# halide/Halide

Measured on AMD Instinct MI355X. Metric: megapixels/sec local_laplacian 8-level fp32 4K, higher is better.
Workload: dtype f32; 1 GPU; apps/local_laplacian J=8 levels=8 alpha=1/7 beta=1, u16 RGB planar 3840x2160; distinct_frames_per_gpu=8, lut_cached=True, streams_per_gpu=4, frame_scheduling=4 frame-queue streams, boundary=C ABI local_laplacian(halide_buffer_t*,int32,float,float,halide_buffer_t*), rccl_ranks=1, parallelism=frames sharded over 1 GPU(s), no data-path collective

## Files before the change

halide_amd/csrc/local_laplacian.hip:

```cpp
#include "hlmi_device_math.h"
#include "hlmi_internal.h"

#include <atomic>
#include <mutex>
#include <optional>
#include <stdlib.h>
#include <string.h>
#include <type_traits>

using namespace hlmi;

namespace {

constexpr int J = 8;
constexpr int MAX_K = 32;
constexpr int STRIP = 126;
constexpr int KCH = 8;
constexpr int D0_THREADS = 256;

struct Level {
    int lox, loy;
    int w, h;
    int ws;
    size_t ps;
// ... 55 lines not shown
    if (i > 2 * half) return;
    float fx = (float)(i - half) * (1.0f / 256.0f);
    lut[i] = (alpha * fx) * dev::halide_exp(((-fx) * fx) * 0.5f);
}

__device__ __forceinline__ int xcd_block() {
    const int nb8 = gridDim.x >> 3, b = blockIdx.x;
    return (b < (nb8 << 3)) ? (b & 7) * nb8 + (b >> 3) : b;
}

__device__ __forceinline__ float down4(float a, float b, float c, float d) {
    return (dev::mad(3.0f, b + c, a) + d) * 0.125f;
}
__device__ __forceinline__ float down4_raw(float a, float b, float c, float d) { return dev::mad(3.0f, b + c, a) + d; }
__device__ __forceinline__ float down4_tail(float a, float b, float c, float d) {
    return (dev::mad(3.0f, b + c, a) + d) * 0.015625f;
}

__device__ __forceinline__ float gray_from(uint16_t r, uint16_t g, uint16_t b) {
    constexpr float s = (float)(1.0 / 65535.0);
    constexpr float C0 = (float)((double)s * (double)0.299f), C1 = (float)((double)s * (double)0.587f),
                    C2 = (float)((double)s * (double)0.114f);
    return dev::mad((float)b, C2, dev::mad2((float)r, C0, (float)g, C1));
}
__device__ __forceinline__ int idx_of(float gray, float Km1, int half) {
    return dev::clampi((int)((gray * Km1) * 256.0f), 0, half);
}
template<bool B1 = false>
__device__ __forceinline__ float g0_val(float gray, float level, float beta, float l) {
    return B1 ? ((gray - level) + level) + l : dev::mad(beta, gray - level, level) + l;
}

__device__ __forceinline__ float lane_prev(float v) {
    return __builtin_bit_cast(float, __builtin_amdgcn_update_dpp(0, __builtin_bit_cast(int, v), 0x138, 0xf, 0xf, true));
}
__device__ __forceinline__ float lane_next(float v) {
    return __builtin_bit_cast(float, __builtin_amdgcn_update_dpp(0, __builtin_bit_cast(int, v), 0x130, 0xf, 0xf, true));
}
__global__ void ll_dpp_probe(int *ok) {
    float v = (float)threadIdx.x;
    float p = lane_prev(v), n = lane_next(v);
    bool good = (threadIdx.x == 0 || p == v - 1.0f) && (threadIdx.x == 63 || n == v + 1.0f);
    unsigned long long m = __ballot(good);
    if (threadIdx.x == 0) *ok = (m == ~0ull) ? 1 : 0;
}

template<bool ODD>
__device__ __forceinline__ float2 hpair(const float (&dy)[4]) {
    if (!ODD) {
        float left = lane_prev(dy[3]);
        float right = lane_next(dy[0]);
        float o0 = down4_tail(left, dy[0], dy[1], dy[2]);
        float o1 = down4_tail(dy[1], dy[2], dy[3], right);
        float o2 = lane_next(o0);
        return make_float2(o1, o2);
    } else {
        float r0 = lane_next(dy[0]), r1 = lane_next(dy[1]);
        float o0 = down4_tail(dy[0], dy[1], dy[2], dy[3]);
        float o1 = down4_tail(dy[2], dy[3], r0, r1);
        return make_float2(o0, o1);
    }
}

struct QuadSel {
    int oq;
    int sel[4];
    bool plain;
};
__device__ __forceinline__ QuadSel quad_sel(int o, int w) {
    QuadSel q;
    q.oq = dev::clampi(o, 0, (w - 1) & ~3);
#pragma unroll
    for (int i = 0; i < 4; i++) q.sel[i] = dev::clampi(o + i, 0, w - 1) - q.oq;
    q.plain = (o >= 0) && (o + 3 <= w - 1);
    return q;
}
template<typename T>
__device__ __forceinline__ T pick4(T x, T y, T z, T w, int s) {
    T lo = (s & 1) ? y : x, hi = (s & 1) ? w : z;
    return (s & 2) ? hi : lo;
}

typedef unsigned short us4_t __attribute__((ext_vector_type(4)));
template<bool NT = false>
__device__ __forceinline__ ushort4 ld_frame4(const uint16_t *p) {
    if (NT) {
        us4_t v = __builtin_nontemporal_load(reinterpret_cast<const us4_t *>(p));
        return make_ushort4(v.x, v.y, v.z, v.w);
    }
    return *reinterpret_cast<const ushort4 *>(p);
}
template<bool NT = false>
__device__ __forceinline__ ushort2 ld_frame2(const void *sbase, uint32_t byte_off) {
    const uint32_t *q = reinterpret_cast<const uint32_t *>(reinterpret_cast<const char *>(sbase) + byte_off);
    const uint32_t w = NT ? __builtin_nontemporal_load(q) : *q;
    return make_ushort2((uint16_t)(w & 0xffffu), (uint16_t)(w >> 16));
}
template<bool NT = false>
__device__ __forceinline__ void st_frame2(void *p, uint16_t a, uint16_t b) {
    const uint32_t w = (uint32_t)a | ((uint32_t)b << 16);
    if (NT) __builtin_nontemporal_store(w, reinterpret_cast<uint32_t *>(p));
    else *reinterpret_cast<uint32_t *>(p) = w;
}

struct Raw {
    ushort4 c0, c1, c2;
};
struct Levels {
    float v[MAX_K];
};

template<bool VEC, bool NT = false>
__device__ __forceinline__ void load_raw(Raw &r, const uint16_t *__restrict__ rp, long co0, long co1, long co2,
                                         int oq, const int (&xo)[4]) {
    if (VEC) {
        r.c0 = ld_frame4<NT>(rp + co0 + oq);
        r.c1 = ld_frame4<NT>(rp + co1 + oq);
        r.c2 = ld_frame4<NT>(rp + co2 + oq);
    } else {
        r.c0 = make_ushort4(rp[co0 + xo[0]], rp[co0 + xo[1]], rp[co0 + xo[2]], rp[co0 + xo[3]]);
        r.c1 = make_ushort4(rp[co1 + xo[0]], rp[co1 + xo[1]], rp[co1 + xo[2]], rp[co1 + xo[3]]);
        r.c2 = make_ushort4(rp[co2 + xo[0]], rp[co2 + xo[1]], rp[co2 + xo[2]], rp[co2 + xo[3]]);
    }
}

template<bool ODD, bool VEC, bool LUT_LDS, bool B1>
__global__ __launch_bounds__(D0_THREADS, 2) void ll_down0(const uint16_t *__restrict__ in, long in_sy, long co0, long co1,
                                                   long co2, Geometry gm, Levels lev, float beta,
                                                   const float *__restrict__ lut_g, float *__restrict__ g1, int Xs,
                                                   int loy1, int w1, int h1, int ws1, size_t ps1, int nsx, int nsy,
                                                   int nunits) {
    extern __shared__ float slut[];
    if (LUT_LDS) {
        for (int i = threadIdx.x; i <= 2 * gm.half; i += D0_THREADS) slut[i] = lut_g[i];
        __syncthreads();
    }
    const float *lut = LUT_LDS ? slut : lut_g;
    const int wave = __builtin_amdgcn_readfirstlane(threadIdx.x >> 6);
    const int unit = xcd_block() * (D0_THREADS / 64) + wave;
    if (unit >= nunits) return;
    const int lane = threadIdx.x & 63;
    const int sy = unit % nsy, sx = unit / nsy;
    const int off = STRIP * sx + 2 * lane;
    const int P = Xs + off;
    const int q0 = ODD ? 2 * P - 1 : 2 * P - 2;
    const int iw = gm.ix1 - gm.ix0 + 1, ih = gm.iy1 - gm.iy0;
    const QuadSel qs = quad_sel(q0 - gm.ix0, iw);
    int xo[4];
#pragma unroll
    for (int i = 0; i < 4; i++) xo[i] = qs.oq + qs.sel[i];
    const bool edge_wave = VEC && __any(!qs.plain);
    const bool store_ok = (lane < 63) && (off < w1);
    const int t0 = (int)((long)sy * h1 / nsy), t1 = (int)((long)(sy + 1) * h1 / nsy) - 1;

    auto row_ptr = [&](int y_abs) -> const uint16_t * {
        return in + (long)(dev::clampi(y_abs - gm.iy0, 0, ih)) * in_sy;
    };

    for (int kb = 0; kb < gm.K; kb += KCH) {
        const int nk = min(KCH, gm.K - kb);
        const bool with_in = (kb == 0);
        const int lbase = gm.half - 256 * (kb + KCH - 1);
        float level[KCH];
#pragma unroll
        for (int kk = 0; kk < KCH; kk++) {
            const float lk = (float)(kb + kk) * gm.inv_Km1;
// ... 353 lines not shown
                level2(kk - 1);
            }
            __builtin_amdgcn_sched_barrier(0);
        }
        state_issue(KCH);
        res[KCH] = hpair<ODD0>(dy[KCH & 1]);
        level2(KCH);
        prep_row(rc, n0);
        prep_row(rd, n1);
        __builtin_amdgcn_sched_barrier(0);
        if (T >= Ts0 && T <= Ts1) {
            float *drow = p.g1 + (size_t)(T - p.loy1) * p.ws1 + off1;
            if (st1_ok) {
#pragma unroll
                for (int kk = 0; kk <= KCH; kk++) *reinterpret_cast<float2 *>(drow + (size_t)kk * p.ps1) = res[kk];
            }
        }
        if (EXCH && pub) {
#pragma unroll
            for (int kk = 0; kk <= KCH; kk++) pub[kk * 64] = res[kk];
        }
        __builtin_amdgcn_sched_barrier(0);
        if (T + 1 < T1) {
            load_row(rc, 2 * T + 5);
            load_row(rd, 2 * T + 6);
        }
        __builtin_amdgcn_sched_barrier(0);
    };
    Row p0, p1, p2, p3;
    prep_row(rc, p0);
    prep_row(rd, p1);
    load_row(rc, 2 * T0 + 3);
    load_row(rd, 2 * T0 + 4);
    LL_PROBE_T(pt2);
    for (int T = T0; T <= T1; T += 2) {
        const bool first = EXCH && T == T0;
        step(std::integral_constant<int, 0>{}, T, p0, p1, p2, p3, a, b, a2, b2, first && publish ? pub_mine : nullptr);
        step(std::integral_constant<int, 1>{}, T + 1, p2, p3, p0, p1, a2, b2, a, b,
             first && publish ? pub_mine + (KCH + 1) * 64 : nullptr);
        if (first) __syncthreads();
#if HLMI_LL_PROBE
        if (first) { LL_PROBE_T(pt3); pr_3 = pt3; }
#endif
    }
    LL_PROBE_T(pt4);
    LL_PROBE_ADD(0, pt1 - pt0); LL_PROBE_ADD(1, 1); LL_PROBE_ADD(2, pt2 - pt1); LL_PROBE_ADD(3, pr_3 - pt2);
    LL_PROBE_ADD(16, pr_a - pr_a0); LL_PROBE_ADD(17, pr_a0 - pt1);
    LL_PROBE_ADD(4, pt4 - pt2); LL_PROBE_ADD(5, (T1 - T0 + 1)); LL_PROBE_ADD(6, pt4 - pt0);
    if (EXCH && !self_halo) {
        float *d2 = p.g2 + (size_t)(B - p.loy2) * p.ws2 + off2;
#pragma unroll
        for (int k = 0; k <= KCH; k++) {
            const float2 sa = st2[(2 * k) * 64], sb = st2[(2 * k + 1) * 64];
            const float2 c = pub_next[k * 64], d = pub_next[(KCH + 1 + k) * 64];
            const float rx = dev::mad(3.0f, sb.x + c.x, sa.x) + d.x, ry = dev::mad(3.0f, sb.y + c.y, sa.y) + d.y;
            float o;
            if (ODD1) {
                const float nx = lane_next(rx), ny = lane_next(ry);
                o = down4_tail(rx, ry, nx, ny);
            } else {
                const float py = lane_prev(ry), nx = lane_next(rx);
                o = down4_tail(py, rx, ry, nx);
            }
            if (st2_ok) d2[(size_t)k * p.ps2] = o;
        }
    }
    };
    if (edge_wave) walk(std::true_type{});
    else walk(std::false_type{});
}

struct D01EArgs {
    D01Args d;
    float *outl0;
    int oy0, oh;
    unsigned nsx_magic;
};
typedef float f2 __attribute__((ext_vector_type(2)));
__device__ __forceinline__ f2 f2s(float v) { return f2{v, v}; }
__device__ __forceinline__ f2 fma2(f2 a, f2 b, f2 c) { return __builtin_elementwise_fma(a, b, c); }
__device__ __forceinline__ f2 mad_2(f2 a, f2 b, f2 c) { return dev::CANON_FMA ? fma2(a, b, c) : a * b + c; }
__device__ __forceinline__ f2 mad2_2(f2 a, f2 b, f2 c, f2 d) { return dev::CANON_FMA ? fma2(a, b, c * d) : a * b + c * d; }

template<bool ODD0, bool ODD1, bool B1, bool EXCH, bool NT>
__global__ __launch_bounds__(D0_THREADS, 2) void ll_down01e(D01EArgs pe, Geometry gm, Levels lev) {
    const D01Args &p = pe.d;
    LL_RESIDENCY(0);
    extern __shared__ float slut[];
    for (int i = threadIdx.x; i <= 2 * gm.half; i += D0_THREADS) slut[i] = p.lut_g[i];
    __syncthreads();
    const int wave = __builtin_amdgcn_readfirstlane(threadIdx.x >> 6);
    const int lane = threadIdx.x & 63;
    int sx, A, B;
    bool self_halo = true;
    bool publish = false;
    if (EXCH) {
        const int wg = xcd_block();
        const int gy = pe.nsx_magic ? (int)__umulhi((unsigned)wg, pe.nsx_magic) : wg;
        sx = wg - gy * p.nsx;
        const int GA = p.loy2 + gy * p.rows_base + min(gy, p.rows_rem);
        const int GB = GA + p.rows_base + (gy < p.rows_rem ? 1 : 0) - 1;
        const int n = (GB - GA + 1 + 1 + 3) >> 2;
        A = GA + wave * n, B = min(A + n - 1, GB);
        if (A > GB) {
            __syncthreads();
            return;
        }
        self_halo = !(wave < 3 && A + n <= GB);
        publish = wave > 0;
    } else {
        const int unit = xcd_block() * (D0_THREADS / 64) + wave;
        if (unit >= p.nunits) return;
        sx = p.nsy_magic ? (int)__umulhi((unsigned)unit, p.nsy_magic) : unit;
        const int sy = unit - sx * p.nsy;
        A = p.loy2 + sy * p.rows_base + min(sy, p.rows_rem);
        B = A + p.rows_base + (sy < p.rows_rem ? 1 : 0) - 1;
    }
    const int P = p.Pbase + 2 * p.S2 * sx + 2 * lane;
    const int q0 = ODD0 ? 2 * P - 1 : 2 * P - 2;
    const int iw = gm.ix1 - gm.ix0 + 1, ih = gm.iy1 - gm.iy0;
    const QuadSel qs = quad_sel(q0 - gm.ix0, iw);
    int xo[4];
#pragma unroll
    for (int i = 0; i < 4; i++) xo[i] = qs.oq + qs.sel[i];
    const bool edge_wave = __any(!qs.plain);
    const int T0 = 2 * A - 1, T1 = self_halo ? 2 * B + 2 : 2 * B;
    const int Ts0 = max(EXCH ? 2 * A - 1 : 2 * A, p.loy1), Ts1 = min(EXCH ? 2 * B : 2 * B + 1, p.loy1 + p.h1 - 1);
    const int off1 = P - p.so1;
    const bool st1_ok = lane < p.S2 && off1 >= 0 && off1 < p.w1;
    const int X2 = ODD1 ? (P + 1) >> 1 : P >> 1;
    const int off2 = X2 - p.so2;
    const bool st2_ok = (ODD1 ? lane < p.S2 : (lane >= 1 && lane <= p.S2)) && off2 >= 0 && off2 < p.w2;
    const bool em_ok = lane >= 1 && lane <= p.S2 && q0 >= gm.ix0 && q0 + 3 <= gm.ix1;
    float *const em_col = pe.outl0 + (q0 - gm.ix0);
    f2 *st2 = reinterpret_cast<f2 *>(slut + ((2 * gm.half + 2) & ~1)) + wave * D01_STATE + lane;
    f2 *pub_all = reinterpret_cast<f2 *>(slut + ((2 * gm.half + 2) & ~1)) + (D0_THREADS / 64) * D01_STATE + lane;
    f2 *pub_mine = pub_all + (wave - 1) * D01_STATE, *pub_next = pub_all + wave * D01_STATE;
    const int lbase = gm.half - 256 * (KCH - 1);
    float level[KCH];
#pragma unroll
    for (int kk = 0; kk < KCH; kk++) {
        level[kk] = lev.v[kk];
        asm volatile("" : "+v"(level[kk]));
    }
    auto walk = [&](auto edge_tag) {
    constexpr bool EDGE = decltype(edge_tag)::value;
    auto load_row = [&](Raw &r, int y_abs) {
        const uint16_t *rp = p.in + (long)(dev::clampi(y_abs - gm.iy0, 0, ih)) * p.in_sy;
        load_raw<true, NT>(r, rp, p.co0, p.co1, p.co2, qs.oq, xo);
    };
    auto u16s = [&](const ushort4 &c, uint16_t (&o)[4]) {
        const uint2 w = __builtin_bit_cast(uint2, c);
        o[0] = (uint16_t)(w.x & 0xffffu), o[1] = (uint16_t)(w.x >> 16);
        o[2] = (uint16_t)(w.y & 0xffffu), o[3] = (uint16_t)(w.y >> 16);
    };
    struct Row {
        f2 g[2];
        int l[4];
    };
    auto prep_row = [&](const Raw &r, Row &o) {
        uint16_t rr[4], gg[4], bb[4];
        u16s(r.c0, rr), u16s(r.c1, gg), u16s(r.c2, bb);
        constexpr float s = (float)(1.0 / 65535.0);
        constexpr float C0 = (float)((double)s * (double)0.299f), C1 = (float)((double)s * (double)0.587f),
                        C2 = (float)((double)s * (double)0.114f);
#pragma unroll
        for (int h = 0; h < 2; h++) {
            const f2 fr = {(float)rr[h], (float)rr[h + 2]}, fg = {(float)gg[h], (float)gg[h + 2]}, fb = {(float)bb[h], (float)bb[h + 2]};
            o.g[h] = mad_2(fb, f2s(C2), mad2_2(fr, f2s(C0), fg, f2s(C1)));
        }
        if (EDGE) {
            const float g0 = o.g[0].x, g1v = o.g[1].x, g2v = o.g[0].y, g3 = o.g[1].y;
            o.g[0].x = pick4(g0, g1v, g2v, g3, qs.sel[0]), o.g[1].x = pick4(g0, g1v, g2v, g3, qs.sel[1]);
            o.g[0].y = pick4(g0, g1v, g2v, g3, qs.sel[2]), o.g[1].y = pick4(g0, g1v, g2v, g3, qs.sel[3]);
        }
#pragma unroll
        for (int h = 0; h < 2; h++) {
            const f2 t = (o.g[h] * gm.Km1) * 256.0f;
            o.l[h] = (min((int)t.x, gm.half) + lbase) * 4;
            o.l[h + 2] = (min((int)t.y, gm.half) + lbase) * 4;
        }
#pragma unroll
        for (int i = 0; i < 4; i++) asm volatile("" : "+v"(o.l[i]));
    };
    auto lut_issue = [&](int kk, const Row &r0, const Row &r1, f2 (&dst)[4]) {
        auto rd = [&](int l) {
            return *reinterpret_cast<const float *>(reinterpret_cast<const char *>(slut) + l + 1024 * (KCH - 1 - kk));
        };
        dst[0].x = rd(r0.l[0]), dst[1].x = rd(r0.l[1]), dst[0].y = rd(r0.l[2]), dst[1].y = rd(r0.l[3]);
        dst[2].x = rd(r1.l[0]), dst[3].x = rd(r1.l[1]), dst[2].y = rd(r1.l[2]), dst[3].y = rd(r1.l[3]);
    };
    auto plane_vals = [&](int kk, const Row &r0, const Row &r1, const f2 (&lv)[4], f2 (&v0)[2], f2 (&v1)[2]) {
        if (B1 && kk == 0) {
            v0[0] = r0.g[0] + lv[0], v0[1] = r0.g[1] + lv[1], v1[0] = r1.g[0] + lv[2], v1[1] = r1.g[1] + lv[3];
        } else if (kk < KCH) {
            const f2 L = f2s(level[kk < KCH ? kk : 0]);
            f2 t[4] = {r0.g[0] - L, r0.g[1] - L, r1.g[0] - L, r1.g[1] - L};
            if (!B1 && !dev::CANON_FMA) {
#pragma unroll
                for (int i = 0; i < 4; i++) t[i] = p.beta * t[i];
            }
#pragma unroll
            for (int i = 0; i < 4; i++) t[i] = (!B1 && dev::CANON_FMA) ? fma2(f2s(p.beta), t[i], L) : t[i] + L;
            v0[0] = t[0] + lv[0], v0[1] = t[1] + lv[1], v1[0] = t[2] + lv[2], v1[1] = t[3] + lv[3];
        } else {
            v0[0] = r0.g[0], v0[1] = r0.g[1], v1[0] = r1.g[0], v1[1] = r1.g[1];
        }
    };
    auto vpass = [&](const f2 (&ia)[2], const f2 (&ib)[2], const f2 (&c)[2], const f2 (&d)[2], f2 (&o)[2]) {
        f2 t[2] = {ib[0] + c[0], ib[1] + c[1]};
        if (dev::CANON_FMA) {
            t[0] = fma2(f2s(3.0f), t[0], ia[0]), t[1] = fma2(f2s(3.0f), t[1], ia[1]);
        } else {
            t[0] = 3.0f * t[0], t[1] = 3.0f * t[1];
            t[0] = ia[0] + t[0], t[1] = ia[1] + t[1];
        }
        o[0] = t[0] + d[0], o[1] = t[1] + d[1];
    };
    auto hpair2 = [&](const f2 (&dy)[2]) {
        const float d4[4] = {dy[0].x, dy[1].x, dy[0].y, dy[1].y};
        const float2 r = hpair<ODD0>(d4);
        return f2{r.x, r.y};
    };
    struct EmPix {
        f2 lut, qa, qb, ta, tb;
        float lif;
    };
    auto em_gather = [&](const Row &n, int i, const f2 *rq, const f2 *rt, EmPix &g) {
        constexpr int COL[4] = {ODD0 ? -1 : -2, -1, ODD0 ? 0 : -1, 0};
        const uint32_t aq0 = (uint32_t)(size_t)rq, at0 = (uint32_t)(size_t)rt, alut = (uint32_t)(size_t)slut + 1024u * (KCH - 2);
        auto rd2 = [](uint32_t addr, auto swap_tag) {
            f2 v;
            if (decltype(swap_tag)::value) asm volatile("ds_read2st64_b32 %0, %1 offset0:4" : "=v"(v) : "v"(addr) : "memory");
            else asm volatile("ds_read2st64_b32 %0, %1 offset1:4" : "=v"(v) : "v"(addr) : "memory");
            return v;
        };
        constexpr std::false_type asc{};
        constexpr std::true_type desc{};
        const int pos = n.l[i] - lbase * 4;
        const int li = min(pos >> 10, KCH - 2);
        const uint32_t po = (uint32_t)(li << 10) + (uint32_t)(COL[i] * 4);
        g.lut = rd2(alut + (uint32_t)n.l[i] - (uint32_t)(li << 10), desc);
        if ((COL[i] & 1) == 0) {
            auto rd64 = [](uint32_t addr, auto plane1) {
                f2 v;
                if (decltype(plane1)::value) asm volatile("ds_read_b64 %0, %1 offset:1024" : "=v"(v) : "v"(addr) : "memory");
                else asm volatile("ds_read_b64 %0, %1" : "=v"(v) : "v"(addr) : "memory");
                return v;
            };
            g.qa = rd64(aq0 + po, asc), g.qb = rd64(aq0 + po, desc);
            g.ta = rd64(at0 + po, asc), g.tb = rd64(at0 + po, desc);
        } else {
            g.qa = rd2(aq0 + po, asc), g.qb = rd2(aq0 + po + 4u, asc);
            g.ta = rd2(at0 + po, asc), g.tb = rd2(at0 + po + 4u, asc);
        }
        g.lif = (float)li;
    };
    auto em_wait = [&](EmPix &g, auto after_tag) {
        constexpr int AFTER = decltype(after_tag)::value;
        static_assert(AFTER >= 0 && AFTER <= 3, "");
        if (AFTER == 0) asm volatile("s_waitcnt lgkmcnt(0)" : "+v"(g.lut), "+v"(g.qa), "+v"(g.qb), "+v"(g.ta), "+v"(g.tb));
        if (AFTER == 1) asm volatile("s_waitcnt lgkmcnt(5)" : "+v"(g.lut), "+v"(g.qa), "+v"(g.qb), "+v"(g.ta), "+v"(g.tb));
        if (AFTER == 2) asm volatile("s_waitcnt lgkmcnt(10)" : "+v"(g.lut), "+v"(g.qa), "+v"(g.qb), "+v"(g.ta), "+v"(g.tb));
        if (AFTER == 3) asm volatile("s_waitcnt lgkmcnt(15)" : "+v"(g.lut), "+v"(g.qa), "+v"(g.qb), "+v"(g.ta), "+v"(g.tb));
    };
    auto em_arith = [&](const Row &n, int i, const EmPix &g, auto yodd_tag) {
        constexpr bool YODD = decltype(yodd_tag)::value;
        const bool xodd = ODD0 ? (i & 1) == 0 : (i & 1) == 1;
        auto hl = [&](f2 fa, f2 fb) {
            if (xodd) return fma2(fb, f2s(0.25f), fa * 0.75f);
            return dev::CANON_FMA ? fma2(fb, f2s(0.75f), fa * 0.25f) : fma2(fa, f2s(0.25f), fb * 0.75f);
        };
        auto vl = [](f2 uq, f2 ut) {
            return (dev::CANON_FMA && !YODD) ? fma2(ut, f2s(0.75f), uq * 0.25f) : fma2(uq, f2s(0.25f), ut * 0.75f);
        };
        const float gr = n.g[i & 1][i >> 1];
        const float lf = gr * gm.Km1 - g.lif;
        const f2 lev = f2{g.lif, g.lif + 1.0f} * gm.inv_Km1;
        constexpr int COLP[4] = {ODD0 ? -1 : -2, -1, ODD0 ? 0 : -1, 0};
        f2 u;
        if ((COLP[i] & 1) == 0) {
            auto hls = [&](float fa, float fb) {
                if (xodd) return __builtin_fmaf(fb, 0.25f, fa * 0.75f);
                return dev::CANON_FMA ? __builtin_fmaf(fb, 0.75f, fa * 0.25f) : __builtin_fmaf(fa, 0.25f, fb * 0.75f);
            };
            auto vls = [](float uq, float ut) {
                return (dev::CANON_FMA && !YODD) ? __builtin_fmaf(ut, 0.75f, uq * 0.25f) : __builtin_fmaf(uq, 0.25f, ut * 0.75f);
            };
            u = f2{vls(hls(g.qa.x, g.qa.y), hls(g.ta.x, g.ta.y)), vls(hls(g.qb.x, g.qb.y), hls(g.tb.x, g.tb.y))};
        } else {
            u = vl(hl(g.qa, g.qb), hl(g.ta, g.tb));
        }
        const f2 g2 = f2s(gr);
        const f2 l = (B1 ? ((g2 - lev) + lev) + g.lut : mad_2(f2s(p.beta), g2 - lev, lev) + g.lut) - u;
        if (dev::CANON_FMA) return __builtin_fmaf(1.0f - lf, l.x, lf * l.y);
        const f2 m = f2{1.0f - lf, lf} * l;
        return m.x + m.y;
    };
    constexpr std::true_type row_odd{};
    constexpr std::false_type row_even{};
    constexpr std::integral_constant<int, 0> after0{};
    constexpr std::integral_constant<int, 1> after1{};
    constexpr std::integral_constant<int, 2> after2{};
    constexpr std::integral_constant<int, 3> after3{};
    auto emit_row = [&](const Row &n, const f2 *rq, const f2 *rt, float (&r)[4], auto yodd_tag) {
        EmPix g[4];
#pragma unroll
        for (int i = 0; i < 4; i++) em_gather(n, i, rq, rt, g[i]);
        em_wait(g[0], after3), r[0] = em_arith(n, 0, g[0], yodd_tag);
        em_wait(g[1], after2), r[1] = em_arith(n, 1, g[1], yodd_tag);
        em_wait(g[2], after1), r[2] = em_arith(n, 2, g[2], yodd_tag);
        em_wait(g[3], after0), r[3] = em_arith(n, 3, g[3], yodd_tag);
    };
    auto emit_store = [&](int y, const float (&r)[4]) {
        if (em_ok && y >= pe.oy0 && y < pe.oy0 + pe.oh) {
            typedef float f4_t __attribute__((ext_vector_type(4)));
            f4_t *const dst = reinterpret_cast<f4_t *>(em_col + (size_t)(y - pe.oy0) * iw);
            if (NT) __builtin_nontemporal_store(f4_t{r[0], r[1], r[2], r[3]}, dst);
            else *dst = f4_t{r[0], r[1], r[2], r[3]};
        }
    };
#if HLMI_LL_PROBE
    unsigned long long pr_planes = 0, pr_emit = 0, pr_prep = 0, pr_steps = 0;
    LL_PROBE_T(pe0);
    const unsigned long long pc0 = __builtin_readcyclecounter();
#endif
    f2 a[KCH + 1][2], b[KCH + 1][2], a2[KCH + 1][2], b2[KCH + 1][2];
    f2 pcr[KCH + 1];
    Raw rc, rd;
    {
        Raw ra, rb;
        load_row(ra, 2 * T0 - 1);
        load_row(rb, 2 * T0);
        load_row(rc, 2 * T0 + 1);
        load_row(rd, 2 * T0 + 2);
        Row r0, r1;
        prep_row(ra, r0);
        prep_row(rb, r1);
        f2 lv[2][4];
        lut_issue(0, r0, r1, lv[0]);
#pragma unroll
        for (int kk = 0; kk <= KCH; kk++) {
            if (kk + 1 < KCH) lut_issue(kk + 1, r0, r1, lv[(kk + 1) & 1]);
            __builtin_amdgcn_sched_barrier(0);
            plane_vals(kk, r0, r1, lv[kk & 1], a[kk], b[kk]);
            __builtin_amdgcn_sched_barrier(0);
        }
    }
    auto step = [&](auto ph_tag, int T, const Row &c0, const Row &c1, Row &n0, Row &n1, f2 (&ia)[KCH + 1][2],
                    f2 (&ib)[KCH + 1][2], f2 (&oa)[KCH + 1][2], f2 (&ob)[KCH + 1][2], f2 *pub) {
        constexpr int PH = decltype(ph_tag)::value;
        f2 lv[2][4], dy[2][2];
        f2 res[KCH + 1];
        f2 sa, sb;
        const bool out2 = PH == 1 && T >= 2 * A + 2;
        float *d2 = p.g2 + (size_t)(((T - 2) >> 1) - p.loy2) * p.ws2 + off2;
        LL_PROBE_T(ps0);
        auto level2 = [&](int k) {
            const f2 c = res[k];
            if (PH == 0) {
                pcr[k] = mad_2(f2s(3.0f), sb + c, sa);
                st2[(2 * k) * 64] = c;
            } else {
                const f2 r = pcr[k] + c;
                float o;
                if (ODD1) {
                    const float nx = lane_next(r.x), ny = lane_next(r.y);
                    o = down4_tail(r.x, r.y, nx, ny);
                } else {
                    const float py = lane_prev(r.y), nx = lane_next(r.x);
                    o = down4_tail(py, r.x, r.y, nx);
                }
                if (out2 && st2_ok) d2[(size_t)k * p.ps2] = o;
                st2[(2 * k + 1) * 64] = c;
            }
        };
        auto state_issue = [&](int k) {
            if (PH == 0) sa = st2[(2 * k) * 64], sb = st2[(2 * k + 1) * 64];
        };
        lut_issue(0, c0, c1, lv[0]);
#pragma unroll
        for (int kk = 0; kk <= KCH; kk++) {
            if (kk > 0) state_issue(kk - 1);
            __builtin_amdgcn_sched_barrier(0);
            if (kk + 1 < KCH) lut_issue(kk + 1, c0, c1, lv[(kk + 1) & 1]);
            __builtin_amdgcn_sched_barrier(0);
            plane_vals(kk, c0, c1, lv[kk & 1], oa[kk], ob[kk]);
            vpass(ia[kk], ib[kk], oa[kk], ob[kk], dy[kk & 1]);
            if (kk > 0) {
                res[kk - 1] = hpair2(dy[(kk - 1) & 1]);
                level2(kk - 1);
            }
            __builtin_amdgcn_sched_barrier(0);
        }
        asm volatile("" ::: "memory");
        __builtin_amdgcn_wave_barrier();
        __builtin_amdgcn_sched_barrier(0);
        f2 *const rowT = st2 + (PH == 0 ? 0 : 64), *const rowP = st2 + (PH == 0 ? 64 : 0);
        const bool st1_row = T >= Ts0 && T <= Ts1;
        const bool em_rows = T >= 2 * A && T <= 2 * B + 1;
        EmPix eg[4];
        if (em_rows) {
#pragma unroll
            for (int i = 0; i < 4; i++) em_gather(n0, i, rowT, rowP, eg[i]);
        }
        __builtin_amdgcn_sched_barrier(0);
        state_issue(KCH);
        res[KCH] = hpair2(dy[KCH & 1]);
        level2(KCH);
        if (EXCH && pub) {
#pragma unroll
            for (int kk = 0; kk <= KCH; kk++) pub[(2 * kk) * 64] = res[kk];
        }
        asm volatile("" ::: "memory");
        __builtin_amdgcn_sched_barrier(0);
        LL_PROBE_T(ps1);
        float2 s0 = make_float2(0.0f, 0.0f), s1 = s0;
        const f2 sK = res[KCH];
        if (st1_row) {
            const int lx = dev::clampi((int)(sK.x * gm.Km1), 0, KCH - 2), ly = dev::clampi((int)(sK.y * gm.Km1), 0, KCH - 2);
            const float *fx = reinterpret_cast<const float *>(rowT) + (lx << 8), *fy = reinterpret_cast<const float *>(rowT) + (ly << 8) + 1;
            s0 = make_float2(fx[0], fy[0]), s1 = make_float2(fx[256], fy[256]);
        }
        float eo[4] = {0.0f, 0.0f, 0.0f, 0.0f}, ee[4] = {0.0f, 0.0f, 0.0f, 0.0f};
        if (em_rows) {
            EmPix fg[4];
            em_wait(eg[0], after3), eo[0] = em_arith(n0, 0, eg[0], row_odd);
            __builtin_amdgcn_sched_barrier(0);
            em_gather(n1, 0, rowP, rowT, fg[0]);
            __builtin_amdgcn_sched_barrier(0);
            em_wait(eg[1], after3), eo[1] = em_arith(n0, 1, eg[1], row_odd);
            __builtin_amdgcn_sched_barrier(0);
            em_gather(n1, 1, rowP, rowT, fg[1]);
            __builtin_amdgcn_sched_barrier(0);
            em_wait(eg[2], after3), eo[2] = em_arith(n0, 2, eg[2], row_odd);
            __builtin_amdgcn_sched_barrier(0);
            em_gather(n1, 2, rowP, rowT, fg[2]);
            __builtin_amdgcn_sched_barrier(0);
            em_wait(eg[3], after3), eo[3] = em_arith(n0, 3, eg[3], row_odd);
            __builtin_amdgcn_sched_barrier(0);
            em_gather(n1, 3, rowP, rowT, fg[3]);
            __builtin_amdgcn_sched_barrier(0);
            em_wait(fg[0], after3), ee[0] = em_arith(n1, 0, fg[0], row_even);
            em_wait(fg[1], after2), ee[1] = em_arith(n1, 1, fg[1], row_even);
            em_wait(fg[2], after1), ee[2] = em_arith(n1, 2, fg[2], row_even);
            em_wait(fg[3], after0), ee[3] = em_arith(n1, 3, fg[3], row_even);
        }
        asm volatile("" ::: "memory");
        __builtin_amdgcn_sched_barrier(0);
        LL_PROBE_T(ps2);
        prep_row(rc, n0);
        prep_row(rd, n1);
        __builtin_amdgcn_sched_barrier(0);
        if (st1_row && st1_ok) {
            float *drow = p.g1 + (size_t)(T - p.loy1) * p.ws1 + off1;
            *reinterpret_cast<float2 *>(drow) = s0;
            *reinterpret_cast<float2 *>(drow + p.ps1) = s1;
            *reinterpret_cast<f2 *>(drow + (size_t)KCH * p.ps1) = sK;
        }
        if (em_rows) {
            emit_store(2 * T - 1, eo);
            emit_store(2 * T, ee);
        }
        __builtin_amdgcn_sched_barrier(0);
        if (T + 1 < T1) {
            load_row(rc, 2 * T + 5);
            load_row(rd, 2 * T + 6);
        }
        __builtin_amdgcn_sched_barrier(0);
#if HLMI_LL_PROBE
        LL_PROBE_T(ps3);
        pr_planes += ps1 - ps0, pr_emit += ps2 - ps1, pr_prep += ps3 - ps2, pr_steps += 1;
#endif
    };
    Row p0, p1, p2, p3;
    prep_row(rc, p0);
    prep_row(rd, p1);
    load_row(rc, 2 * T0 + 3);
    load_row(rd, 2 * T0 + 4);
    for (int T = T0; T <= T1; T += 2) {
        const bool first = EXCH && T == T0;
        step(std::integral_constant<int, 0>{}, T, p0, p1, p2, p3, a, b, a2, b2, first && publish ? pub_mine : nullptr);
        step(std::integral_constant<int, 1>{}, T + 1, p2, p3, p0, p1, a2, b2, a, b, first && publish ? pub_mine + 64 : nullptr);
        if (first) __syncthreads();
    }
#if HLMI_LL_PROBE
    LL_PROBE_T(pe1);
#endif
    if (EXCH && !self_halo) {
        float *d2 = p.g2 + (size_t)(B - p.loy2) * p.ws2 + off2;
#pragma unroll
        for (int k = 0; k <= KCH; k++) {
            const f2 sa = st2[(2 * k) * 64], sb = st2[(2 * k + 1) * 64];
            const f2 c = pub_next[(2 * k) * 64], d = pub_next[(2 * k + 1) * 64];
            const f2 r = mad_2(f2s(3.0f), sb + c, sa) + d;
            float o;
            if (ODD1) {
                const float nx = lane_next(r.x), ny = lane_next(r.y);
                o = down4_tail(r.x, r.y, nx, ny);
            } else {
                const float py = lane_prev(r.y), nx = lane_next(r.x);
                o = down4_tail(py, r.x, r.y, nx);
            }
            if (st2_ok) d2[(size_t)k * p.ps2] = o;
        }
        {
            float eo[4], ee[4];
            emit_row(p2, pub_next, st2 + 64, eo, row_odd);
            emit_row(p3, st2 + 64, pub_next, ee, row_even);
            emit_store(4 * B + 1, eo);
            emit_store(4 * B + 2, ee);
        }
    }
#if HLMI_LL_PROBE
    LL_PROBE_T(pe2);
    LL_PROBE_ADD(27, __builtin_readcyclecounter() - pc0);
    LL_PROBE_ADD(28, pe2 - pe0);
    LL_PROBE_ADD(20, pr_planes); LL_PROBE_ADD(21, pr_emit); LL_PROBE_ADD(22, pr_prep); LL_PROBE_ADD(23, pr_steps);
    LL_PROBE_ADD(24, 1); LL_PROBE_ADD(25, pe1 - pe0); LL_PROBE_ADD(26, pe2 - pe1);
#endif
    };
    if (edge_wave) walk(std::true_type{});
    else walk(std::false_type{});
}

struct StripArgs {
    const float *src;
    int slox, sloy, sw, sh, sws;
    size_t sps;
    float *dst;
    int Xs, dloy, dw, dh, dws;
    size_t dps;
    int nsx, nsy, nunits;
};
template<bool ODD>
__device__ __forceinline__ void down_strip_unit(const StripArgs &a, int unit, int lane) {
    const int sy = unit % a.nsy, rest = unit / a.nsy, sx = rest % a.nsx, plane = rest / a.nsx;
    const int off = STRIP * sx + 2 * lane;
    const int P = a.Xs + off;
    const QuadSel qs = quad_sel((ODD ? 2 * P - 1 : 2 * P - 2) - a.slox, a.sw);
    const bool edge_wave = __any(!qs.plain);
    const bool store_ok = (lane < 63) && (off < a.dw);
    const int t0 = (int)((long)sy * a.dh / a.nsy), t1 = (int)((long)(sy + 1) * a.dh / a.nsy) - 1;
    const float *sp = a.src + (size_t)plane * a.sps + qs.oq;
    float *dp = a.dst + (size_t)plane * a.dps + off;
    auto row = [&](int y_abs) -> float4 {
        float4 v = *reinterpret_cast<const float4 *>(sp + (size_t)dev::clampi(y_abs - a.sloy, 0, a.sh - 1) * a.sws);
        if (edge_wave) {
            v = make_float4(pick4(v.x, v.y, v.z, v.w, qs.sel[0]), pick4(v.x, v.y, v.z, v.w, qs.sel[1]),
                            pick4(v.x, v.y, v.z, v.w, qs.sel[2]), pick4(v.x, v.y, v.z, v.w, qs.sel[3]));
        }
        return v;
    };
    const int T0 = a.dloy + t0;
    float4 ra = row(2 * T0 - 1), rb = row(2 * T0), rc = row(2 * T0 + 1), rd = row(2 * T0 + 2);
    for (int t = t0; t <= t1; t++) {
        const int T = a.dloy + t;
        float4 nc = rc, nd = rd;
        if (t < t1) {
            nc = row(2 * T + 3);
            nd = row(2 * T + 4);
        }
        float dy[4] = {down4_raw(ra.x, rb.x, rc.x, rd.x), down4_raw(ra.y, rb.y, rc.y, rd.y), down4_raw(ra.z, rb.z, rc.z, rd.z),
                       down4_raw(ra.w, rb.w, rc.w, rd.w)};
        float2 o = hpair<ODD>(dy);
        if (store_ok) *reinterpret_cast<float2 *>(dp + (size_t)t * a.dws) = o;
        ra = rc, rb = rd, rc = nc, rd = nd;
    }
}
template<bool ODD>
__global__ __launch_bounds__(256) void ll_down_strip(StripArgs a) {
    const int wave = __builtin_amdgcn_readfirstlane(threadIdx.x >> 6);
    const int unit = xcd_block() * 4 + wave;
    if (unit >= a.nunits) return;
    down_strip_unit<ODD>(a, unit, threadIdx.x & 63);
}

constexpr int S2_RPU = 2;
constexpr int S2_NT = 2 * S2_RPU + 2;
constexpr int S2_NSRC = 2 * S2_NT + 2;
struct Strip2Args {
    const float *src;
    int slox, sloy, sw, sh, sws;
    size_t sps;
    float *g1;
    int so1, loy1, w1, h1, ws1;
    size_t ps1;
// ... 1081 lines not shown
    a.dst = b.g[j + 1], a.Xs = d.lox, a.dloy = d.loy, a.dw = d.w, a.dh = d.h, a.dws = d.ws, a.dps = d.ps;
    a.nsx = d.nsx;
    a.nsy = max(1, min(max(pl.units_strip / cols, (d.h + 31) / 32), max(1, d.h / 2)));
    a.nunits = cols * a.nsy;
    return a;
}
CoarseArgs coarse_args(const LlPlan &pl, const LlBuffers &b, int from) {
    CoarseArgs ca;
    for (int dl = 0; from + dl < J; dl++) {
        const Level &L = pl.lv[from + dl];
        DevLevel &D = ca.lv[dl];
        D.g = b.g[from + dl], D.out = b.outg[from + dl], D.lox = L.lox, D.loy = L.loy, D.w = L.w, D.h = L.h, D.ws = L.ws, D.ps = (unsigned)L.ps;
        D.rx0 = L.rx0, D.ry0 = L.ry0, D.rw = L.rx1 - L.rx0 + 1, D.rh = L.ry1 - L.ry0 + 1;
    }
    ca.K = pl.gm.K, ca.Km1 = pl.gm.Km1;
    return ca;
}
UpArgs up_args(const LlPlan &pl, const LlBuffers &b, int j) {
    const Level &a = pl.lv[j], &c = pl.lv[j + 1];
    UpArgs u;
    u.g = b.g[j], u.ws = a.ws, u.ps = a.ps, u.lox = a.lox, u.loy = a.loy, u.gc = b.g[j + 1], u.outc = b.outg[j + 1], u.cws = c.ws, u.cps = c.ps;
    u.clox = c.lox, u.cloy = c.loy, u.rx0 = a.rx0, u.ry0 = a.ry0, u.rw = a.rx1 - a.rx0 + 1, u.rh = a.ry1 - a.ry0 + 1;
    u.K = pl.gm.K, u.Km1 = pl.gm.Km1, u.out = b.outg[j];
    return u;
}

struct LutKey {
    int device, levels;
    uint32_t alpha_bits;
};
static_assert(sizeof(LutKey) <= DERIVED_KEY_BYTES, "key does not fit an entry");
DerivedCache g_luts(8);


int ll_stage_table(void *uc, const DeviceCtx &ctx, const LlPlan &pl, float alpha, LlBuffers &b, DerivedUse &use) {
    const int nlut = pl.nlut;
    LutKey key;
    memset(&key, 0, sizeof key);
    key.device = ctx.device, key.levels = pl.gm.K;
    memcpy(&key.alpha_bits, &alpha, 4);
    int r = derived_acquire(uc, ctx, g_luts, &key, sizeof key, sizeof(float) * ((size_t)nlut + 64), pl.lut_cache, &use);
    if (r) return r;
    if (use.ptr) b.lut = (float *)use.ptr;
    if (use.fill) {
        HLMI_LAUNCH(uc, "ll_remap_lut", ctx.stream, ll_remap_lut, dim3((nlut + 255) / 256), dim3(256), 0, b.lut, pl.gm.half, alpha);
        use.filled(ctx.stream);
    }
    return 0;
}

int ll_stage_down0(void *uc, const LlPlan &pl, const LlBuffers &b, hipStream_t st) {
    const Geometry &gm = pl.gm;
    const Up0Args &f = pl.u0;
    const Level &d = pl.lv[1], &e = pl.lv[2];
    const int levels = gm.K, iw = gm.ix1 - gm.ix0 + 1;
    Levels lev;
    for (int k = 0; k < MAX_K; k++) lev.v[k] = (float)k * gm.inv_Km1;
    constexpr int WPB = D0_THREADS / 64;
    dim3 block(D0_THREADS);
    const double d0_bytes = 6.0 * iw * (gm.iy1 - gm.iy0 + 1) + 4.0 * (levels + 1) * d.w * d.h;
    if (!pl.d01) {
        dim3 grid((pl.d0.nunits + WPB - 1) / WPB);
        timing_note_bytes(d0_bytes);
        return with_flags([&](auto O, auto V, auto L, auto B) -> int {
            HLMI_LAUNCH(uc, "ll_down0", st, (ll_down0<O.value, V.value, L.value, B.value>), grid, block, pl.d0.lds, f.in, f.in_sy,
                        f.gco[0], f.gco[1], f.gco[2], gm, lev, f.beta, b.lut, b.g[1], d.lox, d.loy, d.w, d.h, d.ws, d.ps, d.nsx,
                        pl.d0.nsy, pl.d0.nunits);
            return 0;
        }, d.odd, pl.vec_in, pl.lut_lds, pl.b1);
    }
    D01Args a;
    a.in = f.in, a.in_sy = f.in_sy, a.co0 = f.gco[0], a.co1 = f.gco[1], a.co2 = f.gco[2], a.beta = f.beta, a.lut_g = b.lut;
    a.g1 = b.g[1], a.so1 = d.lox, a.loy1 = d.loy, a.w1 = d.w, a.h1 = d.h, a.ws1 = d.ws, a.ps1 = d.ps;
    a.g2 = b.g[2], a.so2 = e.lox, a.loy2 = e.loy, a.w2 = e.w, a.h2 = e.h, a.ws2 = e.ws, a.ps2 = e.ps;
    a.S2 = pl.d0.pg.S2, a.Pbase = pl.d0.pg.Pbase, a.nsx = pl.d0.pg.nsx, a.nsy = pl.d0.nsy, a.nunits = pl.d0.nunits;
    a.nsy_magic = a.nsy == 1 ? 0u : (unsigned)((1ull << 32) / (unsigned)a.nsy + 1ull);
    a.rows_base = e.h / a.nsy, a.rows_rem = e.h % a.nsy;
    dim3 grid((a.nunits + WPB - 1) / WPB);
    if (pl.emit) {
        timing_note_bytes(6.0 * iw * (gm.iy1 - gm.iy0 + 1) + 4.0 * iw * f.oh + 4.0 * 3.0 * d.w * d.h + 4.0 * (levels + 1) * e.w * e.h);
        D01EArgs ae;
        ae.d = a, ae.outl0 = b.outl0, ae.oy0 = f.oy0, ae.oh = f.oh;
        ae.nsx_magic = a.nsx == 1 ? 0u : (unsigned)((1ull << 32) / (unsigned)a.nsx + 1ull);
        return with_flags([&](auto O0, auto O1, auto B, auto EX, auto NT) -> int {
            HLMI_LAUNCH(uc, "ll_down01", st, (ll_down01e<O0.value, O1.value, B.value, EX.value, NT.value>), grid, block, pl.d0.lds, ae, gm, lev);
            return 0;
        }, d.odd, e.odd, pl.b1, pl.d0.exch, pl.nt);
    }
    timing_note_bytes(d0_bytes + 4.0 * (levels + 1) * e.w * e.h);
    return with_flags([&](auto O0, auto O1, auto B, auto EX) -> int {
        HLMI_LAUNCH(uc, "ll_down01", st, (ll_down01f<O0.value, O1.value, B.value, EX.value>), grid, block, pl.d0.lds, a, gm, lev);
        return 0;
    }, d.odd, e.odd, pl.b1, pl.d0.exch);
}

int ll_stage_down_rest(void *uc, const LlPlan &pl, const LlBuffers &b, hipStream_t st) {
    const Level *lv = pl.lv;
    const int levels = pl.gm.K, S = pl.S;
    if (pl.strip2) {
        const Level &sl = lv[2], &d = lv[3], &e = lv[4];
        Strip2Args a;
        a.src = b.g[2], a.slox = sl.lox, a.sloy = sl.loy, a.sw = sl.w, a.sh = sl.h, a.sws = sl.ws, a.sps = sl.ps;
        a.g1 = b.g[3], a.so1 = d.lox, a.loy1 = d.loy, a.w1 = d.w, a.h1 = d.h, a.ws1 = d.ws, a.ps1 = d.ps;
        a.g2 = b.g[4], a.so2 = e.lox, a.loy2 = e.loy, a.w2 = e.w, a.h2 = e.h, a.ws2 = e.ws, a.ps2 = e.ps;
        a.S2 = pl.s2.pg.S2, a.Pbase = pl.s2.pg.Pbase, a.nsx = pl.s2.pg.nsx, a.nsy = pl.s2.nsy, a.nunits = pl.s2.nunits;
        timing_note_bytes(4.0 * (levels + 1) * ((double)sl.w * sl.h + (double)d.w * d.h + (double)e.w * e.h));
        dim3 grid((a.nunits + 3) / 4), block(256);
        if (int r = with_flags([&](auto O0, auto O1) -> int {
                HLMI_LAUNCH(uc, "ll_down_strip2:2", st, (ll_down_strip2<O0.value, O1.value>), grid, block, 0, a);
                return 0;
            }, d.odd, e.odd)) return r;
    }
    for (int j = 1; j + 1 < J; j++) {
        if (pl.strip2 && (j == 2 || j == 3)) continue;
        if (j == S) {
            const CoarseArgs ca = coarse_args(pl, b, S);
            long total = 0;
            for (int dl = 1; S + dl < J; dl++) total += (long)(levels + 1) * lv[S + dl].w * lv[S + dl].h;
            const int ntx = (lv[J - 1].w + DM_T - 1) / DM_T, nty = (lv[J - 1].h + DM_T - 1) / DM_T;
            dim3 grid((unsigned)(ntx * nty * (levels + 1))), block(256);
            char nm[32];
            snprintf(nm, sizeof nm, "ll_down_multi:%d", S);
            timing_note_bytes(4.0 * ((double)(levels + 1) * lv[S].w * lv[S].h + (double)total));
            if (J - 1 - S == 4) HLMI_LAUNCH(uc, nm, st, (ll_down_multi<4>), grid, block, 0, ca, ntx, nty);
            else if (J - 1 - S == 3) HLMI_LAUNCH(uc, nm, st, (ll_down_multi<3>), grid, block, 0, ca, ntx, nty);
            else if (J - 1 - S == 2) HLMI_LAUNCH(uc, nm, st, (ll_down_multi<2>), grid, block, 0, ca, ntx, nty);
            else HLMI_LAUNCH(uc, nm, st, (ll_down_multi<1>), grid, block, 0, ca, ntx, nty);
            break;
        }
        if (j == 1 && pl.d01) continue;
        const StripArgs sa = strip_args(pl, b, j);
        dim3 grid((sa.nunits + 3) / 4), block(256);
        char nm[32];
        snprintf(nm, sizeof nm, "ll_down_strip:%d", j);
        timing_note_bytes(4.0 * (levels + 1) * ((double)lv[j].w * lv[j].h + (double)lv[j + 1].w * lv[j + 1].h));
        if (int r = with_flags([&](auto O) -> int {
                HLMI_LAUNCH(uc, nm, st, (ll_down_strip<O.value>), grid, block, 0, sa);
                return 0;
            }, lv[j + 1].odd)) return r;
    }
    return 0;
}

int ll_stage_up_coarse(void *uc, const LlPlan &pl, const LlBuffers &b, hipStream_t st) {
    const Level *lv = pl.lv;
    const int levels = pl.gm.K, SU = pl.SU;
    if (SU < J) {
        const CoarseArgs cu = coarse_args(pl, b, SU);
        const int ntx = (cu.lv[0].rw + UM_T - 1) / UM_T, nty = (cu.lv[0].rh + UM_T - 1) / UM_T;
        dim3 grid((unsigned)(ntx * nty)), block(256);
        char nm[32];
        snprintf(nm, sizeof nm, "ll_up_multi:%d", SU);
        {
            const double px = (double)cu.lv[0].rw * cu.lv[0].rh;
            timing_note_bytes(4.0 * 4.0 * px * (SU + 1 < J ? 4.0 / 3.0 : 1.0));
        }
        switch (J - 1 - SU) {
#define LL_UM(T) case T: HLMI_LAUNCH(uc, nm, st, (ll_up_multi<T>), grid, block, 0, cu, ntx); break;
            LL_UM(1) LL_UM(2) LL_UM(3) LL_UM(4) LL_UM(5) LL_UM(6)
#undef LL_UM
        }
    } else {
        const Level &t = lv[J - 1];
        int rw = t.rx1 - t.rx0 + 1, rh = t.ry1 - t.ry0 + 1;
        HLMI_LAUNCH(uc, "ll_top", st, ll_top, dim3((rw + 63) / 64, rh), dim3(64), 0, b.g[J - 1], t.ws, t.ps, t.lox, t.loy, t.rx0,
                    t.ry0, rw, rh, levels, pl.gm.Km1, b.outg[J - 1]);
    }
    for (int j = min(SU, J - 1) - 1; j >= pl.up_low; j--) {
        const UpArgs ua = up_args(pl, b, j);
        char nm[32];
// ... 205 lines not shown
```

Measured before the change: 117,700 Mpx/s.

## Add steady-state row loop with incremental pointers in fused down01 emit kernel

After: 114,700 Mpx/s. 0.975x the previous value.

```diff
diff --git a/halide_amd/csrc/local_laplacian.hip b/halide_amd/csrc/local_laplacian.hip
--- a/halide_amd/csrc/local_laplacian.hip
+++ b/halide_amd/csrc/local_laplacian.hip
@@ -161,6 +161,12 @@
 }
 
 typedef unsigned short us4_t __attribute__((ext_vector_type(4)));
+template<typename T, typename U>
+__device__ __forceinline__ T *lane_ptr(U *base, uint32_t &byte_off) {
+    typedef typename std::conditional<std::is_const<U>::value, const char, char>::type B;
+    asm volatile("" : "+v"(byte_off));
+    return reinterpret_cast<T *>(reinterpret_cast<B *>(base) + byte_off);
+}
 template<bool NT = false>
 __device__ __forceinline__ ushort4 ld_frame4(const uint16_t *p) {
     if (NT) {
@@ -680,8 +686,8 @@
 __device__ __forceinline__ f2 mad_2(f2 a, f2 b, f2 c) { return dev::CANON_FMA ? fma2(a, b, c) : a * b + c; }
 __device__ __forceinline__ f2 mad2_2(f2 a, f2 b, f2 c, f2 d) { return dev::CANON_FMA ? fma2(a, b, c * d) : a * b + c * d; }
 
-template<bool ODD0, bool ODD1, bool B1, bool EXCH, bool NT>
-__global__ __launch_bounds__(D0_THREADS, 2) void ll_down01e(D01EArgs pe, Geometry gm, Levels lev) {
+template<bool ODD0, bool ODD1, bool B1, bool EXCH, bool NT, bool ONE>
+__global__ __launch_bounds__(D0_THREADS, ONE ? 1 : 2) void ll_down01e(D01EArgs pe, Geometry gm, Levels lev) {
     const D01Args &p = pe.d;
     LL_RESIDENCY(0);
     extern __shared__ float slut[];
@@ -718,9 +724,6 @@
     const int q0 = ODD0 ? 2 * P - 1 : 2 * P - 2;
     const int iw = gm.ix1 - gm.ix0 + 1, ih = gm.iy1 - gm.iy0;
     const QuadSel qs = quad_sel(q0 - gm.ix0, iw);
-    int xo[4];
-#pragma unroll
-    for (int i = 0; i < 4; i++) xo[i] = qs.oq + qs.sel[i];
     const bool edge_wave = __any(!qs.plain);
     const int T0 = 2 * A - 1, T1 = self_halo ? 2 * B + 2 : 2 * B;
     const int Ts0 = max(EXCH ? 2 * A - 1 : 2 * A, p.loy1), Ts1 = min(EXCH ? 2 * B : 2 * B + 1, p.loy1 + p.h1 - 1);
@@ -730,7 +733,11 @@
     const int off2 = X2 - p.so2;
     const bool st2_ok = (ODD1 ? lane < p.S2 : (lane >= 1 && lane <= p.S2)) && off2 >= 0 && off2 < p.w2;
     const bool em_ok = lane >= 1 && lane <= p.S2 && q0 >= gm.ix0 && q0 + 3 <= gm.ix1;
-    float *const em_col = pe.outl0 + (q0 - gm.ix0);
+    uint32_t in_lo = (uint32_t)qs.oq * 2u, d1_lo = (uint32_t)off1 * 4u, d2_lo = (uint32_t)off2 * 4u, em_lo = (uint32_t)(q0 - gm.ix0) * 4u;
+    struct {
+        const uint16_t *in;
+        float *d1, *d2, *em;
+    } sp;
     f2 *st2 = reinterpret_cast<f2 *>(slut + ((2 * gm.half + 2) & ~1)) + wave * D01_STATE + lane;
     f2 *pub_all = reinterpret_cast<f2 *>(slut + ((2 * gm.half + 2) & ~1)) + (D0_THREADS / 64) * D01_STATE + lane;
     f2 *pub_mine = pub_all + (wave - 1) * D01_STATE, *pub_next = pub_all + wave * D01_STATE;
@@ -743,10 +750,12 @@
     }
     auto walk = [&](auto edge_tag) {
     constexpr bool EDGE = decltype(edge_tag)::value;
-    auto load_row = [&](Raw &r, int y_abs) {
-        const uint16_t *rp = p.in + (long)(dev::clampi(y_abs - gm.iy0, 0, ih)) * p.in_sy;
-        load_raw<true, NT>(r, rp, p.co0, p.co1, p.co2, qs.oq, xo);
-    };
+    auto load_row_at = [&](Raw &r, const uint16_t *rp) {
+        r.c0 = ld_frame4<NT>(lane_ptr<const uint16_t>(rp + p.co0, in_lo));
+        r.c1 = ld_frame4<NT>(lane_ptr<const uint16_t>(rp + p.co1, in_lo));
+        r.c2 = ld_frame4<NT>(lane_ptr<const uint16_t>(rp + p.co2, in_lo));
+    };
+    auto load_row = [&](Raw &r, int y_abs) { load_row_at(r, p.in + (long)(dev::clampi(y_abs - gm.iy0, 0, ih)) * p.in_sy); };
     auto u16s = [&](const ushort4 &c, uint16_t (&o)[4]) {
         const uint2 w = __builtin_bit_cast(uint2, c);
         o[0] = (uint16_t)(w.x & 0xffffu), o[1] = (uint16_t)(w.x >> 16);
@@ -910,13 +919,16 @@
         em_wait(g[2], after1), r[2] = em_arith(n, 2, g[2], yodd_tag);
         em_wait(g[3], after0), r[3] = em_arith(n, 3, g[3], yodd_tag);
     };
-    auto emit_store = [&](int y, const float (&r)[4]) {
-        if (em_ok && y >= pe.oy0 && y < pe.oy0 + pe.oh) {
+    auto emit_store_at = [&](float *row, const float (&r)[4]) {
+        if (em_ok) {
             typedef float f4_t __attribute__((ext_vector_type(4)));
-            f4_t *const dst = reinterpret_cast<f4_t *>(em_col + (size_t)(y - pe.oy0) * iw);
+            f4_t *const dst = lane_ptr<f4_t>(row, em_lo);
             if (NT) __builtin_nontemporal_store(f4_t{r[0], r[1], r[2], r[3]}, dst);
             else *dst = f4_t{r[0], r[1], r[2], r[3]};
         }
+    };
+    auto emit_store = [&](int y, const float (&r)[4]) {
+        if (y >= pe.oy0 && y < pe.oy0 + pe.oh) emit_store_at(pe.outl0 + (size_t)(y - pe.oy0) * iw, r);
     };
 #if HLMI_LL_PROBE
     unsigned long long pr_planes = 0, pr_emit = 0, pr_prep = 0, pr_steps = 0;
@@ -945,14 +957,19 @@
             __builtin_amdgcn_sched_barrier(0);
         }
     }
-    auto step = [&](auto ph_tag, int T, const Row &c0, const Row &c1, Row &n0, Row &n1, f2 (&ia)[KCH + 1][2],
+    auto step = [&](auto ph_tag, auto steady_tag, int T, const Row &c0, const Row &c1, Row &n0, Row &n1, f2 (&ia)[KCH + 1][2],
                     f2 (&ib)[KCH + 1][2], f2 (&oa)[KCH + 1][2], f2 (&ob)[KCH + 1][2], f2 *pub) {
         constexpr int PH = decltype(ph_tag)::value;
+        constexpr bool STEADY = decltype(steady_tag)::value;
+        if (STEADY) {
+#pragma unroll
+            for (int kk = 0; kk < KCH; kk++) asm volatile("" : "+v"(level[kk]));
+        }
         f2 lv[2][4], dy[2][2];
         f2 res[KCH + 1];
         f2 sa, sb;
-        const bool out2 = PH == 1 && T >= 2 * A + 2;
-        float *d2 = p.g2 + (size_t)(((T - 2) >> 1) - p.loy2) * p.ws2 + off2;
+        const bool out2 = PH == 1 && (STEADY || T >= 2 * A + 2);
+        float *const d2 = STEADY ? sp.d2 : p.g2 + (size_t)(((T - 2) >> 1) - p.loy2) * p.ws2;
         LL_PROBE_T(ps0);
         auto level2 = [&](int k) {
             const f2 c = res[k];
@@ -969,7 +986,7 @@
                     const float py = lane_prev(r.y), nx = lane_next(r.x);
                     o = down4_tail(py, r.x, r.y, nx);
                 }
-                if (out2 && st2_ok) d2[(size_t)k * p.ps2] = o;
+                if (out2 && st2_ok) *lane_ptr<float>(d2 + (size_t)k * p.ps2, d2_lo) = o;
                 st2[(2 * k + 1) * 64] = c;
             }
         };
@@ -995,8 +1012,8 @@
         __builtin_amdgcn_wave_barrier();
         __builtin_amdgcn_sched_barrier(0);
         f2 *const rowT = st2 + (PH == 0 ? 0 : 64), *const rowP = st2 + (PH == 0 ? 64 : 0);
-        const bool st1_row = T >= Ts0 && T <= Ts1;
-        const bool em_rows = T >= 2 * A && T <= 2 * B + 1;
+        const bool st1_row = STEADY || (T >= Ts0 && T <= Ts1);
+        const bool em_rows = STEADY || (T >= 2 * A && T <= 2 * B + 1);
         EmPix eg[4];
         if (em_rows) {
 #pragma unroll
@@ -1006,7 +1023,7 @@
         state_issue(KCH);
         res[KCH] = hpair2(dy[KCH & 1]);
         level2(KCH);
-        if (EXCH && pub) {
+        if (!STEADY && EXCH && pub) {
 #pragma unroll
             for (int kk = 0; kk <= KCH; kk++) pub[(2 * kk) * 64] = res[kk];
         }
@@ -1050,20 +1067,35 @@
         prep_row(rc, n0);
         prep_row(rd, n1);
         __builtin_amdgcn_sched_barrier(0);
-        if (st1_row && st1_ok) {
-            float *drow = p.g1 + (size_t)(T - p.loy1) * p.ws1 + off1;
-            *reinterpret_cast<float2 *>(drow) = s0;
-            *reinterpret_cast<float2 *>(drow + p.ps1) = s1;
-            *reinterpret_cast<f2 *>(drow + (size_t)KCH * p.ps1) = sK;
-        }
-        if (em_rows) {
-            emit_store(2 * T - 1, eo);
-            emit_store(2 * T, ee);
-        }
-        __builtin_amdgcn_sched_barrier(0);
-        if (T + 1 < T1) {
-            load_row(rc, 2 * T + 5);
-            load_row(rd, 2 * T + 6);
+        if (STEADY) {
+            if (st1_ok) {
+                *lane_ptr<float2>(sp.d1, d1_lo) = s0;
+                *lane_ptr<float2>(sp.d1 + p.ps1, d1_lo) = s1;
+                *lane_ptr<f2>(sp.d1 + (size_t)KCH * p.ps1, d1_lo) = sK;
+            }
+            emit_store_at(sp.em, eo);
+            emit_store_at(sp.em + iw, ee);
+            __builtin_amdgcn_sched_barrier(0);
+            load_row_at(rc, sp.in);
+            load_row_at(rd, sp.in + p.in_sy);
+            sp.d1 += p.ws1, sp.em += 2 * iw, sp.in += 2 * p.in_sy;
+            if (PH == 1) sp.d2 += p.ws2;
+        } else {
+            if (st1_row && st1_ok) {
+                float *const drow = p.g1 + (size_t)(T - p.loy1) * p.ws1;
+                *lane_ptr<float2>(drow, d1_lo) = s0;
+                *lane_ptr<float2>(drow + p.ps1, d1_lo) = s1;
+                *lane_ptr<f2>(drow + (size_t)KCH * p.ps1, d1_lo) = sK;
+            }
+            if (em_rows) {
+                emit_store(2 * T - 1, eo);
+                emit_store(2 * T, ee);
+            }
+            __builtin_amdgcn_sched_barrier(0);
+            if (T + 1 < T1) {
+                load_row(rc, 2 * T + 5);
+                load_row(rd, 2 * T + 6);
+            }
         }
         __builtin_amdgcn_sched_barrier(0);
 #if HLMI_LL_PROBE
@@ -1076,17 +1108,31 @@
     prep_row(rd, p1);
     load_row(rc, 2 * T0 + 3);
     load_row(rd, 2 * T0 + 4);
+    const int Tq0 = max(max(T0 + 2, Ts0), max((pe.oy0 + 2) >> 1, (gm.iy0 - 4) >> 1)) | 1;
+    const int Tq1 = min(min(min(2 * B, Ts1 - 1), T1 - 3), min((pe.oy0 + pe.oh - 3) >> 1, (gm.iy0 + ih - 8) >> 1));
+    sp.in = p.in + (long)(2 * Tq0 + 5 - gm.iy0) * p.in_sy;
+    sp.d1 = p.g1 + (long)(Tq0 - p.loy1) * p.ws1;
+    sp.d2 = p.g2 + (long)(((Tq0 - 1) >> 1) - p.loy2) * p.ws2;
+    sp.em = pe.outl0 + (long)(2 * Tq0 - 1 - pe.oy0) * iw;
+    constexpr std::integral_constant<int, 0> ph0{};
+    constexpr std::integral_constant<int, 1> ph1{};
     for (int T = T0; T <= T1; T += 2) {
         const bool first = EXCH && T == T0;
-        step(std::integral_constant<int, 0>{}, T, p0, p1, p2, p3, a, b, a2, b2, first && publish ? pub_mine : nullptr);
-        step(std::integral_constant<int, 1>{}, T + 1, p2, p3, p0, p1, a2, b2, a, b, first && publish ? pub_mine + 64 : nullptr);
+        step(ph0, std::false_type{}, T, p0, p1, p2, p3, a, b, a2, b2, first && publish ? pub_mine : nullptr);
+        step(ph1, std::false_type{}, T + 1, p2, p3, p0, p1, a2, b2, a, b, first && publish ? pub_mine + 64 : nullptr);
         if (first) __syncthreads();
+        if (ONE && !EDGE && T + 2 == Tq0) {
+            for (; T + 2 <= Tq1; T += 2) {
+                step(ph0, std::true_type{}, T + 2, p0, p1, p2, p3, a, b, a2, b2, nullptr);
+                step(ph1, std::true_type{}, T + 3, p2, p3, p0, p1, a2, b2, a, b, nullptr);
+            }
+        }
     }
 #if HLMI_LL_PROBE
     LL_PROBE_T(pe1);
 #endif
     if (EXCH && !self_halo) {
-        float *d2 = p.g2 + (size_t)(B - p.loy2) * p.ws2 + off2;
+        float *const d2 = p.g2 + (size_t)(B - p.loy2) * p.ws2;
 #pragma unroll
         for (int k = 0; k <= KCH; k++) {
             const f2 sa = st2[(2 * k) * 64], sb = st2[(2 * k + 1) * 64];
@@ -1100,7 +1146,7 @@
                 const float py = lane_prev(r.y), nx = lane_next(r.x);
                 o = down4_tail(py, r.x, r.y, nx);
             }
-            if (st2_ok) d2[(size_t)k * p.ps2] = o;
+            if (st2_ok) *lane_ptr<float>(d2 + (size_t)k * p.ps2, d2_lo) = o;
         }
         {
             float eo[4], ee[4];
@@ -2348,10 +2394,10 @@
         D01EArgs ae;
         ae.d = a, ae.outl0 = b.outl0, ae.oy0 = f.oy0, ae.oh = f.oh;
         ae.nsx_magic = a.nsx == 1 ? 0u : (unsigned)((1ull << 32) / (unsigned)a.nsx + 1ull);
-        return with_flags([&](auto O0, auto O1, auto B, auto EX, auto NT) -> int {
-            HLMI_LAUNCH(uc, "ll_down01", st, (ll_down01e<O0.value, O1.value, B.value, EX.value, NT.value>), grid, block, pl.d0.lds, ae, gm, lev);
+        return with_flags([&](auto O0, auto O1, auto B, auto EX, auto NT, auto ONE) -> int {
+            HLMI_LAUNCH(uc, "ll_down01", st, (ll_down01e<O0.value, O1.value, B.value, EX.value, NT.value, ONE.value>), grid, block, pl.d0.lds, ae, gm, lev);
             return 0;
-        }, d.odd, e.odd, pl.b1, pl.d0.exch, pl.nt);
+        }, d.odd, e.odd, pl.b1, pl.d0.exch, pl.nt, pl.d0.lds > 80 * 1024);
     }
     timing_note_bytes(d0_bytes + 4.0 * (levels + 1) * e.w * e.h);
     return with_flags([&](auto O0, auto O1, auto B, auto EX) -> int {
```
